# biointec/columba

Hardware: AMD Instinct MI355X
Metric: reads/sec (150bp, k=4 edit, human ref) (higher is better)
Workload: dtype u64

## Files before the change

### columba_amd/csrc/columba_amd.hip

```cpp
#include "../../include/columba_amd.h"
#include "host_sam.hpp"
#include "host_schemes.hpp"
#include "kernels.hpp"

#include <chrono>
#include <cstring>
#include <functional>
#include <memory>
#include <mutex>
#include <thread>
#include <string>
#include <vector>

using namespace cmb;

static thread_local std::string g_err;
static int fail(int code, const std::string& msg) {
    g_err = msg;
    return code;
}
namespace cmb {
int failWith(int code, const std::string& msg) { return fail(code, msg); }
}
#define HIPCHK(expr)                                                                                  \
    do {                                                                                              \
        hipError_t _e = (expr);                                                                       \
        if (_e != hipSuccess) throw std::runtime_error(std::string(#expr) + ": " + hipGetErrorString(_e)); \
    } while (0)

template <typename T> struct DevBuf {
    T* p = nullptr;
    size_t n = 0;
    DevBuf() {}
    DevBuf(const DevBuf&) = delete;
    DevBuf& operator=(const DevBuf&) = delete;
    ~DevBuf() { release(); }
    void release() {
        if (p) (void)hipFree(p);
        p = nullptr;
        n = 0;
    }
    void alloc(size_t count) {
        release();
        if (count == 0) count = 1;
        HIPCHK(hipMalloc((void**)&p, count * sizeof(T)));
        n = count;
    }
    void upload(const T* h, size_t count) {
        alloc(count);
        if (count) HIPCHK(hipMemcpy(p, h, count * sizeof(T), hipMemcpyHostToDevice));
    }
    void uploadPadded(const T* h, size_t count, size_t pad) {
        alloc(count + pad);
        if (count) HIPCHK(hipMemcpy(p, h, count * sizeof(T), hipMemcpyHostToDevice));
        HIPCHK(hipMemset(p + count, 0, pad * sizeof(T)));
    }
    size_t bytes() const { return n * sizeof(T); }
};

template <typename T> struct PinnedBuf {
    T* p = nullptr;
    size_t cap = 0, n = 0;
    PinnedBuf() {}
    PinnedBuf(const PinnedBuf&) = delete;
    PinnedBuf& operator=(const PinnedBuf&) = delete;
    ~PinnedBuf() {
        if (p) (void)hipHostFree(p);
    }
    void resize(size_t count) {
        if (count > cap) {
            if (p) (void)hipHostFree(p);
            p = nullptr;
            cap = 0;
            const size_t want = count + count / 4 + 64;
            HIPCHK(hipHostMalloc((void**)&p, want * sizeof(T), hipHostMallocDefault));
            cap = want;
        }
        n = count;
    }
    size_t size() const { return n; }
    bool empty() const { return n == 0; }
    T* data() { return p; }
    const T* data() const { return p; }
};

struct cmb_index {
    int device = 0;
    uint32_t saSparseness = 0;
    DevIndex d{};
    DevBuf<uint4> blkF, blkR;
    DevBuf<uint32_t> saSamples;
    DevBuf<uint8_t> text;
    DevBuf<uint32_t> text2;
    DevBuf<uint4> kmer;
    std::vector<uint32_t> seqStarts;
    DevBuf<uint32_t> seqStartsDev;
    uint32_t nSeqsDev = 0;
    uint64_t bytes = 0;
    bool textOnly = false;
    void uploadSeqStarts() {
        std::vector<uint32_t> v = seqStarts;
        if (v.size() < 2) v = {0u, d.n ? d.n - 1u : 0u};
        seqStartsDev.upload(v.data(), v.size());
        nSeqsDev = (uint32_t)v.size() - 1u;
    }
};

#ifdef CMB_BFS_STATS
extern "C" int cmb_debug_bfs_stats(unsigned long long* out, int reset) {
    if (out && hipMemcpyFromSymbol(out, HIP_SYMBOL(cmb::g_bfsStats), 16 * sizeof(unsigned long long)) != hipSuccess) return -1;
    if (reset) {
        unsigned long long z[16] = {};
        if (hipMemcpyToSymbol(HIP_SYMBOL(cmb::g_bfsStats), z, sizeof(z)) != hipSuccess) return -1;
    }
    return 0;
}
#endif
#ifdef CMB_BOUNDS
extern "C" int cmb_debug_oob(unsigned long long* out) {
    return hipMemcpyFromSymbol(out, HIP_SYMBOL(cmb::g_oob), 4 * sizeof(unsigned long long)) == hipSuccess ? 0 : -1;
}
#endif
#ifdef CMB_STAGE_STATS
extern "C" int cmb_debug_stage_stats(unsigned long long* out, int reset) {
    if (out && hipMemcpyFromSymbol(out, HIP_SYMBOL(cmb::g_stageStats), 24 * sizeof(unsigned long long)) != hipSuccess) return -1;
    if (reset) {
        unsigned long long z[24] = {};
        if (hipMemcpyToSymbol(HIP_SYMBOL(cmb::g_stageStats), z, sizeof(z)) != hipSuccess) return -1;
    }
    return 0;
}
#endif
extern "C" const char* cmb_last_error(void) { return g_err.c_str(); }
extern "C" const char* cmb_version(void) { return "columba_amd 0.1 (gfx950)"; }

static void useDevice(int device) { HIPCHK(hipSetDevice(device)); }

static int probeIndex(cmb_index* ix) {
    DevBuf<uint32_t> bad;
    bad.alloc(1);
    HIPCHK(hipMemset(bad.p, 0, sizeof(uint32_t)));
    const uint32_t nProbe = std::min<uint32_t>(ix->d.n, 1u << 20);
    if (!nProbe) return CMB_OK;
    hipLaunchKernelGGL(k_check_index, dim3((nProbe + 255) / 256), dim3(256), 0, 0, ix->d, ix->saSparseness, nProbe, (uint32_t)std::min<size_t>(ix->saSamples.n, 0xFFFFFFFFu), bad.p);
    HIPCHK(hipGetLastError());
    uint32_t hb = 0;
    HIPCHK(hipMemcpy(&hb, bad.p, sizeof(uint32_t), hipMemcpyDeviceToHost));
    if (hb)
        return fail(CMB_ERR_INVALID, "the index arrays do not belong together: " + std::to_string(hb) + " of " + std::to_string(nProbe) +
                                         " probed suffix-array rows do not reach a sampled row within " + std::to_string(ix->saSparseness) +
                                         " LF steps (wrong sparseness, or bit vectors / samples / BWT of different texts)");
    return CMB_OK;
}
extern "C" int cmb_index_validate(cmb_index* idx) {
    if (!idx) return fail(CMB_ERR_INVALID, "null argument");
    try {
        useDevice(idx->device);
        return probeIndex(idx);
    } catch (const std::exception& e) {
        return fail(CMB_ERR_DEVICE, e.what());
    }
}

extern "C" int cmb_index_create(const cmb_index_desc* desc, int device, cmb_index** out) {
    if (!desc || !out) return fail(CMB_ERR_INVALID, "null argument");
    if (desc->text_length == 0 || desc->text_length >= 0xFFFFFFFFull)
        return fail(CMB_ERR_UNSUPPORTED, "text length must fit a 32-bit length_t");
    if (desc->kmer_size > 15) return fail(CMB_ERR_INVALID, "k-mer size > 15 (the reference's -K option takes 0 ... 15, alignparameters.cpp:449)");
    if (desc->sa_sparseness == 0 || (desc->sa_sparseness & (desc->sa_sparseness - 1)))
        return fail(CMB_ERR_INVALID, "suffix array sparseness must be a power of two");
    try {
        int ndev = 0;
        if (hipGetDeviceCount(&ndev) != hipSuccess || ndev == 0)
            return fail(CMB_ERR_DEVICE, "no HIP device available (the product path has no CPU fallback)");
        useDevice(device);
        std::unique_ptr<cmb_index> ix(new cmb_index());
        ix->device = device;
        ix->saSparseness = desc->sa_sparseness;
        const uint64_t n = desc->text_length, N = n + 1;
        const uint64_t bvW = 4 * ((N + 63) / 64), cW = 8 * ((N + 511) / 512);
        const uint64_t nBlocks = N / RANK_BLOCK + 1;
        for (int dir = 0; dir < 2; dir++) {
            DevBuf<uint64_t> bv, cnt;
            bv.upload(dir ? desc->bv_rev : desc->bv_fwd, bvW);
            cnt.upload(dir ? desc->cnt_rev : desc->cnt_fwd, cW);
            DevBuf<uint4>& blk = dir ? ix->blkR : ix->blkF;
            blk.alloc(nBlocks * 2);
            hipLaunchKernelGGL(k_relayout, dim3((unsigned)((nBlocks + 255) / 256)), dim3(256), 0, 0, bv.p, cnt.p, N,
                               nBlocks, blk.p);
            HIPCHK(hipGetLastError());
            HIPCHK(hipDeviceSynchronize());
        }
        const uint64_t saW = (n + 63) / 64;
        {
            DevBuf<uint64_t> bv, cnt;
            bv.upload(desc->sa_bv, saW);
            cnt.upload(desc->sa_bv_counts, (saW + 7) / 4);
            hipLaunchKernelGGL(k_relayout_sa, dim3((unsigned)((nBlocks + 255) / 256)), dim3(256), 0, 0, bv.p, cnt.p, saW,
                               nBlocks, ix->blkF.p);
            HIPCHK(hipGetLastError());
            HIPCHK(hipDeviceSynchronize());
        }
        ix->saSamples.upload(desc->sa_samples, desc->n_samples);
        constexpr uint64_t TEXT_PAD = 640;
        static_assert(TEXT_PAD >= (uint64_t)VROWS + 64, "text padding must cover the longest verification window");
        ix->text.alloc(n + TEXT_PAD);
        HIPCHK(hipMemset(ix->text.p, 0, n + TEXT_PAD));
        HIPCHK(hipMemcpy(ix->text.p, desc->text, n, hipMemcpyHostToDevice));
        hipLaunchKernelGGL(k_encode_text, dim3(4096), dim3(256), 0, 0, ix->text.p, n, n + TEXT_PAD);
        HIPCHK(hipGetLastError());
        bool packedOk = false;
        {
            const uint64_t nWords = (n + TEXT_PAD) / 16;
            ix->text2.alloc(nWords + 16);
            HIPCHK(hipMemset(ix->text2.p, 0, (nWords + 16) * sizeof(uint32_t)));
            DevBuf<uint32_t> bad;
            bad.alloc(1);
            HIPCHK(hipMemset(bad.p, 0, sizeof(uint32_t)));
            hipLaunchKernelGGL(k_pack_text, dim3(4096), dim3(256), 0, 0, ix->text.p, n, nWords, ix->text2.p, bad.p);
            HIPCHK(hipGetLastError());
            uint32_t hb = 0;
            HIPCHK(hipMemcpy(&hb, bad.p, sizeof(uint32_t), hipMemcpyDeviceToHost));
            packedOk = hb == 0 && !getenv("CMB_TEXT_BYTES");
            if (!packedOk) ix->text2.release();
        }
        ix->kmer.alloc(1ull << (2 * desc->kmer_size));
        if (desc->seq_starts) ix->seqStarts.assign(desc->seq_starts, desc->seq_starts + desc->n_seqs);
        DevIndex& d = ix->d;
        d.n = (uint32_t)n;
        for (int i = 0; i < 5; i++) d.counts[i] = (uint32_t)desc->counts[i];
        d.fwd = DevBWT{ix->blkF.p, (uint32_t)desc->dollar_pos_fwd};
        d.rev = DevBWT{ix->blkR.p, (uint32_t)desc->dollar_pos_rev};
        d.saSamples = ix->saSamples.p;
        d.text = ix->text.p;
        d.text2 = packedOk ? ix->text2.p : nullptr;
        d.kmer = ix->kmer.p;
        d.kmerSize = desc->kmer_size;
        d.switchPoint = desc->in_text_switch;
        const uint32_t total = 1u << (2 * desc->kmer_size);
        hipLaunchKernelGGL(k_kmer_table, dim3((total + 255) / 256), dim3(256), 0, 0, d, ix->kmer.p);
        HIPCHK(hipGetLastError());
        HIPCHK(hipDeviceSynchronize());
        if (int rc = probeIndex(ix.get())) return rc;
        ix->bytes = ix->blkF.bytes() + ix->blkR.bytes() + ix->saSamples.bytes() + ix->text.bytes() + ix->text2.bytes() + ix->kmer.bytes();
        ix->uploadSeqStarts();
        *out = ix.release();
        return CMB_OK;
    } catch (const std::exception& e) {
        return fail(CMB_ERR_DEVICE, e.what());
    }
}
namespace {
struct ArrayRef {
    void** p;
    size_t* n;
    size_t elem;
};
inline void indexArrays(cmb_index* ix, ArrayRef out[CMB_DEV_ARRAYS]) {
    out[0] = {(void**)&ix->blkF.p, &ix->blkF.n, sizeof(uint4)};
    out[1] = {(void**)&ix->blkR.p, &ix->blkR.n, sizeof(uint4)};
    out[2] = {(void**)&ix->saSamples.p, &ix->saSamples.n, sizeof(uint32_t)};
    out[3] = {(void**)&ix->text.p, &ix->text.n, sizeof(uint8_t)};
    out[4] = {(void**)&ix->text2.p, &ix->text2.n, sizeof(uint32_t)};
    out[5] = {(void**)&ix->kmer.p, &ix->kmer.n, sizeof(uint4)};
}
inline void bindDevIndex(cmb_index* ix) {
    DevIndex& d = ix->d;
    d.fwd.blk = ix->blkF.p;
    d.rev.blk = ix->blkR.p;
    d.saSamples = ix->saSamples.p;
    d.text = ix->text.p;
    d.text2 = ix->text2.n ? ix->text2.p : nullptr;
    d.kmer = ix->kmer.p;
}
}

extern "C" int cmb_index_layout_of(const cmb_index* idx, cmb_index_layout* out) {
    if (!idx || !out) return fail(CMB_ERR_INVALID, "null argument");
    memset(out, 0, sizeof(*out));
    out->text_length = idx->d.n;
    for (int i = 0; i < 5; i++) out->counts[i] = idx->d.counts[i];
    out->dollar_pos_fwd = idx->d.fwd.dollarPos;
    out->dollar_pos_rev = idx->d.rev.dollarPos;
    out->n_samples = idx->saSamples.n;
    out->sa_sparseness = idx->saSparseness;
    out->kmer_size = idx->d.kmerSize;
    out->in_text_switch = idx->d.switchPoint;
    out->n_seqs = (uint32_t)idx->seqStarts.size();
    ArrayRef a[CMB_DEV_ARRAYS];
    indexArrays(const_cast<cmb_index*>(idx), a);
    for (int i = 0; i < CMB_DEV_ARRAYS; i++) out->bytes[i] = *a[i].p ? (uint64_t)(*a[i].n * a[i].elem) : 0;
    return CMB_OK;
}
extern "C" int cmb_index_seq_starts(const cmb_index* idx, uint32_t* out) {
    if (!idx || (!out && !idx->seqStarts.empty())) return fail(CMB_ERR_INVALID, "null argument");
    if (!idx->seqStarts.empty()) memcpy(out, idx->seqStarts.data(), idx->seqStarts.size() * sizeof(uint32_t));
    return CMB_OK;
}
extern "C" int cmb_index_create_text_only(const char* text, uint64_t n, const uint32_t* seq_starts, uint32_t n_seqs, int device,
                                          cmb_index** out) {
    if (!text || !out) return fail(CMB_ERR_INVALID, "null argument");
    if (n == 0 || n >= 0xFFFFFF00ull) return fail(CMB_ERR_UNSUPPORTED, "text length must fit a 32-bit length_t");
    try {
        useDevice(device);
        std::unique_ptr<cmb_index> ix(new cmb_index());
        ix->device = device;
        ix->textOnly = true;
        constexpr uint64_t TEXT_PAD = 640;
        ix->text.alloc(n + TEXT_PAD);
        HIPCHK(hipMemset(ix->text.p, 0, n + TEXT_PAD));
        HIPCHK(hipMemcpy(ix->text.p, text, n, hipMemcpyHostToDevice));
        hipLaunchKernelGGL(k_encode_text, dim3(4096), dim3(256), 0, 0, ix->text.p, n, n + TEXT_PAD);
        const uint64_t nWords = (n + TEXT_PAD) / 16;
        ix->text2.alloc(nWords + 16);
        HIPCHK(hipMemset(ix->text2.p, 0, (nWords + 16) * sizeof(uint32_t)));
        DevBuf<uint32_t> bad;
        bad.alloc(1);
        HIPCHK(hipMemset(bad.p, 0, sizeof(uint32_t)));
        hipLaunchKernelGGL(k_pack_text, dim3(4096), dim3(256), 0, 0, ix->text.p, n, nWords, ix->text2.p, bad.p);
        HIPCHK(hipGetLastError());
        uint32_t hb = 0;
        HIPCHK(hipMemcpy(&hb, bad.p, sizeof(uint32_t), hipMemcpyDeviceToHost));
        if (hb) ix->text2.release();
        if (seq_starts && n_seqs) ix->seqStarts.assign(seq_starts, seq_starts + n_seqs);
        ix->d.n = (uint32_t)n;
        ix->d.text = ix->text.p;
        ix->d.text2 = hb ? nullptr : ix->text2.p;
        ix->uploadSeqStarts();
        ix->bytes = ix->text.bytes() + ix->text2.bytes();
        *out = ix.release();
        return CMB_OK;
    } catch (const std::exception& e) {
        return fail(CMB_ERR_DEVICE, e.what());
    }
}

extern "C" int cmb_index_create_empty(const cmb_index_layout* L, const uint32_t* seq_starts, int device, cmb_index** out) {
    if (!L || !out) return fail(CMB_ERR_INVALID, "null argument");
    if (L->text_length == 0 || L->text_length >= 0xFFFFFFFFull || L->kmer_size > 15)
        return fail(CMB_ERR_INVALID, "index layout out of range");
    try {
        int ndev = 0;
        if (hipGetDeviceCount(&ndev) != hipSuccess || ndev == 0)
            return fail(CMB_ERR_DEVICE, "no HIP device available (the product path has no CPU fallback)");
        useDevice(device);
        std::unique_ptr<cmb_index> ix(new cmb_index());
        ix->device = device;
        ix->saSparseness = L->sa_sparseness;
        ArrayRef a[CMB_DEV_ARRAYS];
        indexArrays(ix.get(), a);
        {
            const uint64_t n = L->text_length, rankBytes = ((n + 1) / RANK_BLOCK + 1) * 2 * sizeof(uint4);
            if (L->sa_sparseness == 0 || (L->sa_sparseness & (L->sa_sparseness - 1)))
// ... 2433 lines not shown
```

### columba_amd/csrc/dev_index.hpp

```cpp
#pragma once
#include <hip/hip_runtime.h>
#include <stdint.h>

namespace cmb {

struct DevBWT {
    const uint4* blk;
    uint32_t dollarPos;
};

struct DevIndex {
    uint32_t n;
    uint32_t counts[5];
    DevBWT fwd, rev;
    const uint32_t* saSamples;
    const uint8_t* text;
    const uint32_t* text2;
    const uint4* kmer;
    uint32_t kmerSize;
    uint32_t switchPoint;
};

struct Range {
    uint32_t b, e;
    __host__ __device__ bool empty() const { return e <= b; }
    __host__ __device__ uint32_t width() const { return e <= b ? 0u : e - b; }
};
struct RangePair {
    Range sa, rev;
    __host__ __device__ bool empty() const { return sa.empty(); }
    __host__ __device__ uint32_t width() const { return sa.width(); }
};

constexpr uint32_t RANK_BLOCK = 32;

struct RankChunks {
    uint4 abs, bits;
    uint32_t bit;
};
__device__ __forceinline__ void loadRankChunks(const DevBWT& t, uint32_t p, RankChunks& k) {
    const uint4* B = t.blk + (size_t)(p >> 5) * 2;
    k.bit = p & 31u;
    k.abs = B[0];
    k.bits = B[1];
}
__device__ __forceinline__ void ranksFromChunks(const RankChunks& k, uint32_t p, uint32_t dollarPos, uint32_t R[4]) {
    const uint32_t lowmask = (1u << k.bit) - 1u;
    R[0] = k.abs.x + (uint32_t)__popc(k.bits.x & lowmask);
    R[1] = k.abs.y + (uint32_t)__popc(k.bits.y & lowmask);
    R[2] = k.abs.z + (uint32_t)__popc(k.bits.z & lowmask);
    R[3] = p - (p > dollarPos ? 1u : 0u);
}

__device__ __forceinline__ void loadRankChunksRaw(const DevBWT& t, uint32_t p, uint4 v[2]) {
    const uint4* B = t.blk + (size_t)(p >> 5) * 2;
    v[0] = B[0];
    v[1] = B[1];
}
__device__ __forceinline__ void loadRankPairRaw(const DevBWT& t, uint32_t pb, uint32_t pe, uint4 v[4]) {
    const uint32_t blkB = pb >> 5, blkE = pe >> 5;
    const uint4* B = t.blk + (size_t)blkB * 2;
    const uint4* E = t.blk + (size_t)blkE * 2;
    v[0] = B[0];
    v[1] = B[1];
    v[2] = v[3] = make_uint4(0u, 0u, 0u, 0u);
    if (blkE != blkB) {
        v[2] = E[0];
        v[3] = E[1];
    }
}
__device__ __forceinline__ void rankPairEnd(const uint4 v[4], uint32_t pb, uint32_t pe, uint4 w[2]) {
    const bool same = (pb >> 5) == (pe >> 5);
    w[0] = same ? v[0] : v[2];
    w[1] = same ? v[1] : v[3];
}
__device__ __forceinline__ void ranksFromRaw(const uint4 v[2], uint32_t p, uint32_t dollarPos, uint32_t R[4]) {
    const uint32_t lowmask = (1u << (p & 31u)) - 1u;
    R[0] = v[0].x + (uint32_t)__popc(v[1].x & lowmask);
    R[1] = v[0].y + (uint32_t)__popc(v[1].y & lowmask);
    R[2] = v[0].z + (uint32_t)__popc(v[1].z & lowmask);
    R[3] = p - (p > dollarPos ? 1u : 0u);
}

__device__ __forceinline__ void rank4(const DevBWT& t, uint32_t p, uint32_t R[4]) {
    RankChunks k;
    loadRankChunks(t, p, k);
    ranksFromChunks(k, p, t.dollarPos, R);
}

__device__ __forceinline__ uint64_t rank1(const DevBWT& t, uint32_t c, uint64_t p) {
    uint32_t R[4];
    rank4(t, (uint32_t)p, R);
    return R[c];
}

__device__ __forceinline__ uint32_t rankRefLayout(const uint64_t* bv, const uint64_t* cnt, uint32_t c, uint64_t p,
                                                  uint64_t N) {
    uint32_t extra = 0;
// ... 39 lines not shown
    r2.e = s + x + r1.width();
    if (mode == 1) {
        child.sa = r1;
        child.rev = r2;
    } else {
        child.sa = r2;
        child.rev = r1;
    }
    return !child.sa.empty();
}

__device__ __forceinline__ bool childFromRanksFlat(const DevIndex& ix, int mode, const RangePair& p, uint32_t c, const uint32_t Rb[4],
                                                   const uint32_t Re[4], uint32_t db, uint32_t de, RangePair& child) {
    const uint32_t start = ix.counts[c];
    const uint32_t b1 = occFromR(Rb, c) + start, e1 = occFromR(Re, c) + start;
    const uint32_t w1 = e1 > b1 ? e1 - b1 : 0u;
    const uint32_t x = cumFromR(Re, c, de) - cumFromR(Rb, c, db);
    const uint32_t b2 = (mode == 1 ? p.rev.b : p.sa.b) + x, e2 = b2 + w1;
    const bool fwd = mode == 0, uni = mode == 2;
    child.sa.b = fwd ? b2 : b1;
    child.sa.e = fwd ? e2 : e1;
    child.rev.b = uni ? 0u : fwd ? b1 : b2;
    child.rev.e = uni ? 0u : fwd ? e1 : e2;
    return e1 > b1;
}

__device__ __forceinline__ void loadExtendRanks(const DevIndex& ix, int mode, const RangePair& p,
                                                uint32_t Rb[4], uint32_t Re[4], uint32_t& db,
                                                uint32_t& de) {
    DevBWT t = ix.fwd;
    Range tr = p.sa;
    if (mode == 0) {
        t = ix.rev;
        tr = p.rev;
    }
    uint4 v[4], w[2];
    loadRankPairRaw(t, tr.b, tr.e, v);
    rankPairEnd(v, tr.b, tr.e, w);
    ranksFromRaw(v, tr.b, t.dollarPos, Rb);
    ranksFromRaw(w, tr.e, t.dollarPos, Re);
    db = tr.b > t.dollarPos ? 1u : 0u;
    de = tr.e > t.dollarPos ? 1u : 0u;
}

__device__ __forceinline__ bool extendOne(const DevIndex& ix, int mode, const RangePair& p, uint32_t c,
                                          RangePair& child) {
    uint32_t Rb[4], Re[4], db, de;
    loadExtendRanks(ix, mode, p, Rb, Re, db, de);
    return childFromRanks(ix, mode, p, c, Rb, Re, db, de, child);
}

__device__ __forceinline__ bool rowSampled(const RankChunks& k) { return (k.bits.w >> k.bit) & 1u; }
__device__ __forceinline__ uint32_t sampleIndex(const RankChunks& k) {
    return k.abs.w + (uint32_t)__popc(k.bits.w & ((1u << k.bit) - 1u));
}
__device__ __forceinline__ bool saMarked(const DevIndex& ix, uint32_t row) {
    RankChunks k;
    loadRankChunks(ix.fwd, row, k);
    return rowSampled(k);
}
__device__ __forceinline__ uint32_t saRank(const DevIndex& ix, uint32_t row) {
    RankChunks k;
    loadRankChunks(ix.fwd, row, k);
    return sampleIndex(k);
}

__device__ __forceinline__ uint32_t lfFromChunks(const DevIndex& ix, const RankChunks& ch, uint32_t k) {
    if (k == ix.fwd.dollarPos) {
        return ix.counts[0];
    }
    uint32_t R[4];
    ranksFromChunks(ch, k, ix.fwd.dollarPos, R);
    const uint32_t bit = ch.bit;
    const uint32_t c = ((ch.bits.x >> bit) & 1u) ? 1u : ((ch.bits.y >> bit) & 1u) ? 2u : ((ch.bits.z >> bit) & 1u) ? 3u : 4u;
    return ix.counts[c] + occFromR(R, c);
}
__device__ __forceinline__ uint32_t findLF(const DevIndex& ix, uint32_t k) {
    if (k == ix.fwd.dollarPos) return ix.counts[0];
    RankChunks ch;
    loadRankChunks(ix.fwd, k, ch);
    return lfFromChunks(ix, ch, k);
}

__device__ __forceinline__ uint32_t findSA(const DevIndex& ix, uint32_t row, uint32_t* lf) {
    uint32_t l = 0;
    RankChunks ch;
    loadRankChunks(ix.fwd, row, ch);
    while (!rowSampled(ch)) {
        row = lfFromChunks(ix, ch, row);
        loadRankChunks(ix.fwd, row, ch);
        l++;
    }
    if (lf) *lf += l;
    return ix.saSamples[sampleIndex(ch)] + l;
}

}
```

### columba_amd/csrc/kernels.hpp

```cpp
#pragma once
#include "dev_partition.hpp"
#include <cstring>
#include <rocprim/device/device_radix_sort.hpp>
#include <rocprim/device/device_scan.hpp>
#include <rocprim/device/device_run_length_encode.hpp>

namespace cmb {

__global__ void k_rank(DevIndex ix, int rev, const uint32_t* __restrict__ c, const uint64_t* __restrict__ p,
                       uint64_t n, uint64_t* __restrict__ out) {
    const uint64_t i = (uint64_t)blockIdx.x * blockDim.x + threadIdx.x;
    if (i >= n) return;
    out[i] = rank1(rev ? ix.rev : ix.fwd, c[i], p[i]);
}

__device__ __forceinline__ uint32_t rank9RefLayout(const uint64_t* bv, const uint64_t* cnt, uint64_t nWords, uint64_t p) {
    uint64_t w = p >> 6, b = p & 63;
    if (nWords == 0) return 0;
    if (w >= nWords) {
        w = nWords - 1;
        b = 64;
    }
    uint64_t rv = cnt[(w >> 3) * 2];
    const uint32_t sub = (uint32_t)(w & 7u);
    if (sub) rv += (cnt[(w >> 3) * 2 + 1] >> ((sub - 1u) * 9u)) & 0x1FFull;
    const uint64_t lowmask = b >= 64 ? ~0ull : b ? (~0ull >> (64 - b)) : 0ull;
    return (uint32_t)rv + (uint32_t)__popcll((unsigned long long)(bv[w] & lowmask));
}

__global__ void k_relayout(const uint64_t* __restrict__ bv, const uint64_t* __restrict__ cnt, uint64_t N,
                           uint64_t nBlocks, uint4* __restrict__ out) {
    const uint64_t blk = (uint64_t)blockIdx.x * blockDim.x + threadIdx.x;
    if (blk >= nBlocks) return;
    const uint64_t nWords = (N + 63) / 64;
    const uint64_t w = blk >> 1;
    const uint32_t sh = (uint32_t)(blk & 1u) * 32u;
    uint32_t bits[3];
    for (uint32_t c = 0; c < 3; c++) bits[c] = w < nWords ? (uint32_t)(bv[w * 4 + c] >> sh) : 0u;
    uint4 abs;
    abs.x = rankRefLayout(bv, cnt, 0, blk * RANK_BLOCK, N);
    abs.y = rankRefLayout(bv, cnt, 1, blk * RANK_BLOCK, N);
    abs.z = rankRefLayout(bv, cnt, 2, blk * RANK_BLOCK, N);
    abs.w = 0;
    out[blk * 2] = abs;
    out[blk * 2 + 1] = make_uint4(bits[0], bits[1], bits[2], 0u);
}

__global__ void k_relayout_sa(const uint64_t* __restrict__ saBv, const uint64_t* __restrict__ saCnt, uint64_t saWords, uint64_t nBlocks,
                              uint4* __restrict__ out) {
    const uint64_t blk = (uint64_t)blockIdx.x * blockDim.x + threadIdx.x;
    if (blk >= nBlocks) return;
    const uint64_t w = blk >> 1;
    const uint32_t sh = (uint32_t)(blk & 1u) * 32u;
    reinterpret_cast<uint32_t*>(out + blk * 2)[3] = rank9RefLayout(saBv, saCnt, saWords, blk * RANK_BLOCK);
    reinterpret_cast<uint32_t*>(out + blk * 2 + 1)[3] = w < saWords ? (uint32_t)(saBv[w] >> sh) : 0u;
}

__global__ void __launch_bounds__(256)
k_extend(DevIndex ix, int mode, const uint4* __restrict__ in, uint64_t n, uint4* __restrict__ out,
         uint8_t* __restrict__ ok) {
    for (uint64_t i = (uint64_t)blockIdx.x * blockDim.x + threadIdx.x; i < n;
         i += (uint64_t)gridDim.x * blockDim.x) {
        const uint4 v = in[i];
        RangePair p{{v.x, v.y}, {v.z, v.w}};
        uint32_t Rb[4], Re[4], db, de;
        loadExtendRanks(ix, mode, p, Rb, Re, db, de);
        uint32_t okbits = 0;
#pragma unroll
        for (uint32_t ch = 1; ch <= 4; ch++) {
            RangePair child;
            const bool o = childFromRanks(ix, mode, p, ch, Rb, Re, db, de, child);
            out[i * 4 + (ch - 1)] = make_uint4(child.sa.b, child.sa.e, child.rev.b, child.rev.e);
            okbits |= (o ? 1u : 0u) << (8 * (ch - 1));
        }
        reinterpret_cast<uint32_t*>(ok)[i] = okbits;
    }
}

__global__ void k_locate(DevIndex ix, const uint32_t* __restrict__ rows, uint64_t n, uint32_t* __restrict__ out,
                         unsigned long long* lfTotal) {
    const uint64_t i = (uint64_t)blockIdx.x * blockDim.x + threadIdx.x;
    if (i >= n) return;
    uint32_t lf = 0;
    out[i] = findSA(ix, rows[i], &lf);
    if (lf) atomicAdd(lfTotal, (unsigned long long)lf);
}

__global__ void k_check_index(DevIndex ix, uint32_t maxSteps, uint32_t nProbe, uint32_t nSamples, uint32_t* __restrict__ bad) {
    const uint32_t i = blockIdx.x * blockDim.x + threadIdx.x;
    if (i >= nProbe) return;
    uint32_t row = (uint32_t)(((uint64_t)i * ix.n) / nProbe);
    for (uint32_t l = 0;; l++) {
        if (row >= ix.n) break;
        RankChunks ch;
        loadRankChunks(ix.fwd, row, ch);
        if (rowSampled(ch)) {
            const uint32_t si = sampleIndex(ch);
            if (si < nSamples && (uint64_t)ix.saSamples[si] + l < ix.n) return;
            break;
        }
        if (l == maxSteps) break;
        row = lfFromChunks(ix, ch, row);
    }
    atomicAdd(bad, 1u);
}

__global__ void k_kmer_table(DevIndex ix, uint4* __restrict__ table) {
    const uint32_t key = blockIdx.x * blockDim.x + threadIdx.x;
    const uint32_t total = 1u << (2 * ix.kmerSize);
    if (key >= total) return;
    RangePair r{{0, ix.n}, {0, ix.n}};
    bool ok = true;
    for (int i = (int)ix.kmerSize - 1; i >= 0 && ok; i--) {
        const uint32_t code = ((key >> (2 * i)) & 3u) + 1u;
        RangePair child;
        ok = extendOne(ix, 0, r, code, child);
        r = child;
    }
    table[key] = ok ? make_uint4(r.sa.b, r.sa.e, r.rev.b, r.rev.e) : make_uint4(0, 0, 0, 0);
}

struct __attribute__((packed, aligned(1))) Unaligned16 {
    uint32_t x, y, z, w;
};
struct __attribute__((packed, aligned(1))) Unaligned8 {
    uint32_t x, y;
};
__device__ __forceinline__ uint4 loadText16(const uint8_t* p) {
    const Unaligned16 v = *reinterpret_cast<const Unaligned16*>(p);
    return make_uint4(v.x, v.y, v.z, v.w);
}
__global__ void __launch_bounds__(256)
k_prep(const uint8_t* __restrict__ reads, const uint64_t* __restrict__ offs, uint32_t nReads, uint32_t maxLen,
       uint32_t gw, uint32_t chunks, uint8_t* __restrict__ seq, uint32_t* __restrict__ G, uint32_t* __restrict__ rec,
       uint32_t recW) {
    const uint32_t gid = blockIdx.x * blockDim.x + threadIdx.x;
    const uint32_t r = gid / chunks, w = gid % chunks;
    if (r >= nReads) return;
    const uint8_t* rd = reads + offs[r];
    const uint32_t len = (uint32_t)(offs[r + 1] - offs[r]);
    if (len > maxLen) return;
    if (32 * w >= len) {
        if (w == 0 && rec) {
            rec[(size_t)(2 * r) * recW] = 0;
            rec[(size_t)(2 * r + 1) * recW] = 0;
        }
        return;
    }
    uint32_t fA[4] = {0, 0, 0, 0}, fB[4] = {0, 0, 0, 0};
    uint8_t* sF = seq + (size_t)(2 * r) * maxLen;
    uint8_t* sR = seq + (size_t)(2 * r + 1) * maxLen;
    const uint32_t nT = min(32u, len - 32 * w);
    uint32_t cF[8] = {0, 0, 0, 0, 0, 0, 0, 0}, cR[8] = {0, 0, 0, 0, 0, 0, 0, 0};
    uint32_t wa[8], wb[8];
    {
        const uint4 x = loadText16(rd + 32 * w), y = loadText16(rd + 32 * w + 16);
        wa[0] = x.x, wa[1] = x.y, wa[2] = x.z, wa[3] = x.w, wa[4] = y.x, wa[5] = y.y, wa[6] = y.z, wa[7] = y.w;
    }
    if (offs[r] + len >= 32ull * w + 32ull) {
        const uint8_t* pb = rd + len - 32 * w - 32;
        const uint4 x = loadText16(pb), y = loadText16(pb + 16);
        wb[0] = x.x, wb[1] = x.y, wb[2] = x.z, wb[3] = x.w, wb[4] = y.x, wb[5] = y.y, wb[6] = y.z, wb[7] = y.w;
    } else {
#pragma unroll
        for (uint32_t j = 0; j < 8; j++) wb[j] = 0;
#pragma unroll
        for (uint32_t t = 0; t < 32; t++)
            if (t < nT) wb[(31u - t) >> 2] |= (uint32_t)rd[len - 1 - 32 * w - t] << (8u * ((31u - t) & 3u));
// ... 544 lines not shown
            nxt = loadText16(tp + 16 * (c + 2));
        }
    }
    if (!STORE && i > firstRow) {
        const uint32_t e1 = edPrev;
        if (e1 <= maxED && e1 >= minED && e1 <= edPrev2) centreMask |= 1u << (i - 1 - firstRow);
    }
    return i;
}

constexpr uint32_t VK_LOW = 10;
__host__ __device__ __forceinline__ uint32_t windowEnd(uint32_t maxEnd, uint32_t start, uint32_t m) {
    const unsigned long long e = (unsigned long long)start + m - 1ull;
    return e < maxEnd ? (uint32_t)e : maxEnd;
}
__host__ __device__ __forceinline__ unsigned long long packVerifyKey(uint32_t rs, uint32_t start, uint32_t maxED,
                                                                     uint32_t minED, uint32_t fixed) {
    return ((unsigned long long)rs << 39) | ((unsigned long long)(maxED & 7u) << 36) | ((unsigned long long)(minED & 7u) << 33) |
           ((unsigned long long)(fixed & 1u) << 32) | (unsigned long long)((start >> VK_LOW) | (start << (32u - VK_LOW)));
}
__host__ __device__ __forceinline__ uint32_t verifyKeyStart(unsigned long long key) {
    const uint32_t v = (uint32_t)key;
    return (v << VK_LOW) | (v >> (32u - VK_LOW));
}
constexpr uint32_t VKW_RS = 41;
__host__ __device__ __forceinline__ unsigned long long packVerifyKeyW(uint32_t rs, uint32_t start, uint32_t maxED, uint32_t minED,
                                                                      uint32_t fixed) {
    return ((unsigned long long)rs << VKW_RS) | ((unsigned long long)(maxED & 15u) << 37) | ((unsigned long long)(minED & 15u) << 33) |
           ((unsigned long long)(fixed & 1u) << 32) | (unsigned long long)((start >> VK_LOW) | (start << (32u - VK_LOW)));
}

__device__ __forceinline__ bool verifyEdit(const DevIndex& ix, const uint64_t* offs, const MFull& mf,
                                           uint32_t rs, uint32_t start, uint32_t maxED, uint32_t minED, uint32_t fixed,
                                           uint32_t mult, uint32_t& cStarted, uint32_t& cRows, uint32_t& cText,
                                           uint32_t& cAbort, uint32_t& cCig, uint4& tbRec, uint64_t* Ml,
                                           uint32_t limitEnd = 0 ) {
    cStarted += mult;
    const uint32_t len = (uint32_t)(offs[(rs >> 1) + 1] - offs[rs >> 1]);
    const uint32_t nZeros = fixed ? 1u : 2u * maxED + 1u;
    MatGeom g;
    g.n = len + 1;
    g.maxED = maxED;
    g.Wv = nZeros - 1 + maxED;
    g.Wh = maxED;
    g.m = max(g.Wv + g.n, g.Wv + g.Wh + 1u);
    const uint32_t maxEnd = ix.n - 1;
    const uint32_t hEnd = limitEnd ? min(maxEnd, limitEnd) : windowEnd(maxEnd, start, g.m);
    const uint32_t size = hEnd > start ? hEnd - start : 0;
    if (!g.inFinalColumn(size)) return false;
    uint32_t mask = 0, rows = 0;
    uint64_t edPack, edPackHi;
    const VPlanes noPlanes{nullptr, 0, 0};
    const uint32_t i = forwardPass<false>(ix, mf, rs, g, nZeros, start, size, maxED, minED,
                                          mask, edPack, edPackHi, noPlanes, 0, rows, Ml);
    cRows += rows * mult;
    cText += rows * mult;
    if (i <= size - g.sfc() || mask == 0) {
        cAbort += mult;
        return false;
    }
    cCig += (uint32_t)__popc(mask) * mult;
    tbRec = make_uint4(rs, start, mask, maxED | (fixed << 4));
    return true;
}

__device__ __forceinline__ uint32_t mismatch4(uint32_t tw, uint32_t sw) {
    const uint32_t x = (tw + 0x01010101u) ^ sw;
    return ((x | (x >> 1) | (x >> 2)) | (tw >> 2)) & 0x01010101u;
}
__device__ __forceinline__ uint32_t mismatch16(const uint4& t, const uint4& r, uint32_t nC, uint32_t m[4]) {
    const uint32_t tw[4] = {t.x, t.y, t.z, t.w}, sw[4] = {r.x, r.y, r.z, r.w};
    uint32_t cnt = 0;
#pragma unroll
    for (uint32_t w = 0; w < 4; w++) {
        const uint32_t nb = nC > 4 * w ? min(4u, nC - 4 * w) : 0u;
        const uint32_t valid = nb >= 4u ? 0x01010101u : (0x01010101u & ((1u << (8u * nb)) - 1u));
        m[w] = mismatch4(tw[w], sw[w]) & valid;
        cnt += (uint32_t)__popc(m[w]);
    }
    return cnt;
}

template <bool KEYS>
__global__ void __launch_bounds__(256)
k_verify(DevIndex ix, const uint64_t* __restrict__ offs, uint32_t maxLen, uint32_t gw,
         const uint8_t* __restrict__ seq, MFull mf, const uint4* __restrict__ items,
         uint32_t nItems, uint4* __restrict__ tbq, uint32_t tbCap, unsigned long long* __restrict__ vkeys, Queues q,
         uint32_t wideKeys = 0 ) {
    __shared__ uint64_t Ml[ML_WORDS];
    const uint32_t slot = blockIdx.x * blockDim.x + threadIdx.x;
    uint32_t cLF = 0, cLoc = 0, cText = 0, cRows = 0, cAbort = 0, cCig = 0, cStarted = 0, cRep = 0, flags = 0;
    WaveChunk chT, chB;
    bool ovT = false, ovB = false;
    auto holeT = [&](uint32_t i) { q.text[i].rsId = 0xFFFFFFFFu; };
    auto holeB = [&](uint32_t i) { tbq[i] = make_uint4(0, 0, 0, 0); };
    const uint32_t stride = gridDim.x * blockDim.x;
    const uint32_t waveBase = slot & ~63u;
    const VPlanes noPlanes{nullptr, 0, 0};
    for (uint32_t base = waveBase; base < nItems; base += stride) {
        const uint32_t it = base + (threadIdx.x & 63u);
        uint32_t nOut = 0, nTb = 0;
        uint4 outRec = make_uint4(0, 0, 0, 0), tbRec = make_uint4(0, 0, 0, 0);
        uint32_t rs = 0;
        unsigned long long vkey = ~0ull;
        uint4 item = make_uint4(0xFFFFFFFFu, 0, 0, 0);
        if (it < nItems) item = items[it];
        if (item.x != 0xFFFFFFFFu) {
            rs = item.x;
            const uint32_t row = item.y, a = item.z, meta = item.w;
            const uint32_t kind = (meta >> 21) & 3u;
            const uint32_t maxED = (meta >> 12) & 15u, minED = (meta >> 16) & 15u;
            const uint32_t fixed = (meta >> 20) & 1u;
            const uint32_t shift = meta & 0xFFFu;
            const uint32_t len = (uint32_t)(offs[(rs >> 1) + 1] - offs[rs >> 1]);
            const uint8_t* s = seq + (size_t)rs * maxLen;
            uint32_t pos;
            if ((meta >> 23) & 1u) {
                pos = row;
            } else {
                cLoc++;
                pos = findSA(ix, row, &cLF);
            }
            if (kind == ITEM_EXACT) {
                if (fixed) {
                    outRec = make_uint4(pos, pos + len, 0, 0);
                    nOut = 1;
                } else {
                    cStarted++;
                    const uint32_t remaining = a;
                    bool ok = pos >= remaining;
                    const uint32_t p0 = pos - remaining;
                    for (uint32_t j = 0; ok && j < remaining; j += 16) {
                        const uint32_t nC = min(16u, remaining - j);
                        uint32_t m[4];
                        const uint32_t cnt = mismatch16(loadText16(ix.text + p0 + j), *reinterpret_cast<const uint4*>(s + j), nC, m);
                        if (cnt == 0) {
                            cText += nC;
                        } else {
                            const uint32_t w = m[0] ? 0u : m[1] ? 1u : m[2] ? 2u : 3u;
                            const uint32_t mw = w == 0 ? m[0] : w == 1 ? m[1] : w == 2 ? m[2] : m[3];
                            cText += 4 * w + (((uint32_t)__ffs(mw) - 1u) >> 3) + 1u;
                            ok = false;
                        }
                    }
                    if (ok) {
                        outRec = make_uint4(p0, p0 + len, 0, 0);
                        nOut = 1;
                    } else {
                        cAbort++;
                    }
                }
            } else if (kind == ITEM_HAMMING) {
                cStarted++;
                const uint32_t lengthBefore = a;
                const uint32_t Tb = pos > lengthBefore ? pos - lengthBefore : 0;
                const uint32_t Te = Tb + len;
                if ((unsigned long long)Tb + len <= ix.n) {
                    uint32_t score = 0;
                    for (uint32_t j = 0; j < len; j += 16) {
                        const uint32_t nC = min(16u, len - j);
                        uint32_t m[4];
                        const uint32_t cnt = mismatch16(loadText16(ix.text + Tb + j), *reinterpret_cast<const uint4*>(s + j), nC, m);
                        if (score + cnt <= maxED) {
                            score += cnt;
                            cText += nC;
                            continue;
                        }
                        for (uint32_t t = 0; t < nC; t++) {
                            const uint32_t mw = (t >> 2) == 0 ? m[0] : (t >> 2) == 1 ? m[1] : (t >> 2) == 2 ? m[2] : m[3];
                            cText++;
                            score += (mw >> (8u * (t & 3u))) & 1u;
                            if (score > maxED) break;
                        }
                        break;
                    }
                    if (score <= maxED && score >= minED) {
                        outRec = make_uint4(Tb, Te, score, 0);
                        nOut = 1;
                    }
                }
            } else {
                const bool direct = (meta >> 23) & 1u;
                const uint32_t startDiff = direct ? 0u : a;
                const uint32_t sum = pos + shift;
                const uint32_t start = sum >= startDiff ? sum - startDiff : 0;
                if (KEYS) {
                    vkey = wideKeys ? packVerifyKeyW(rs, start, maxED, minED, fixed) : packVerifyKey(rs, start, maxED, minED, fixed);
                } else if (verifyEdit(ix, offs, mf, rs, start, maxED, minED, fixed, 1u, cStarted, cRows, cText, cAbort,
                                      cCig, tbRec, Ml, direct ? a : 0u)) {
                    nTb = 1;
                }
            }
        }
        if (KEYS && it < nItems) vkeys[it] = vkey;
        cRep += nOut;
        const uint32_t o1 = chT.alloc(&q.cnt[2], q.textCap, nOut, 256u, ovT, holeT);
        if (nOut && o1 != 0xFFFFFFFFu) q.text[o1] = TextOccRec{rs, outRec.x, outRec.y, outRec.z};
        const uint32_t o2 = chB.alloc(&q.cnt[7], tbCap, nTb, 256u, ovB, holeB);
        if (nTb && o2 != 0xFFFFFFFFu) tbq[o2] = tbRec;
    }
    chT.fill(holeT);
    chB.fill(holeB);
    if (ovT) flags |= FLAG_TEXT_OVERFLOW;
    if (ovB) flags |= FLAG_CAPACITY;
// ... 122 lines not shown
            if (!__any(have)) {
                if (__all(done)) break;
                turn = 0xFFFFFFFFu;
                continue;
            }
            if (have) mx.loadBlock(ix, G, gw, rs, len, start, r >> 4);
            skip = fresh;
            if (fresh) r = 1u;
        }
        bool survives = false;
        if (have && !skip) {
            uint64_t M, D0;
            const bool valid = mx.step(g, r, M, D0);
            rows++;
            if (!valid || r == size) {
                const uint32_t i = valid ? r : r - 1u;
                if (i <= size - g.sfc()) {
                    cStarted += mult;
                    cRows += rows * mult;
                    cAbort += mult;
                } else {
                    survives = true;
                }
                have = false;
            } else {
                r++;
            }
        }
        if (__any(survives)) {
            const uint32_t o = chS.alloc(&work[1], listCap, survives ? 1u : 0u, 256u, ovS, holeS);
            if (survives && o != 0xFFFFFFFFu) list[o] = u;
        }
    }
    chS.fill(holeS);
    if (ovS) flags |= FLAG_CAPACITY;
    const uint32_t local[8] = {0u, 0u, cRows, cRows, cAbort, 0u, cStarted, 0u};
    const int which[8] = {8, 9, 10, 11, 3, 4, 2, 1};
    flushCounters(q, local, which, 8);
    if (flags) atomicOr(&q.cnt[3], flags);
}

template <bool KEYED, class WX>
__global__ void __launch_bounds__(256)
k_verify_wide(DevIndex ix, const uint64_t* __restrict__ offs, uint32_t maxLen, const uint8_t* __restrict__ seq, const uint32_t* __restrict__ G,
              uint32_t gw, const uint4* __restrict__ items, uint32_t nItems, const unsigned long long* __restrict__ ukeys,
              const uint32_t* __restrict__ counts, const uint32_t* __restrict__ list, const uint32_t* __restrict__ nList,
              uint8_t* __restrict__ slab, uint32_t slotBytes, Queues q) {
    const uint32_t slot = blockIdx.x * blockDim.x + threadIdx.x, nSlots = gridDim.x * blockDim.x, lane = threadIdx.x & 63u;
    uint4* const rowBits = reinterpret_cast<uint4*>(slab + (size_t)(slot - lane) * slotBytes) + lane;
    auto putRow = [&](uint32_t r, uint64_t a, uint64_t b) {
        rowBits[(size_t)r * 64u] = make_uint4((uint32_t)a, (uint32_t)(a >> 32), (uint32_t)b, (uint32_t)(b >> 32));
    };
    uint32_t cLF = 0, cLoc = 0, cRows = 0, cAbort = 0, cCig = 0, cStarted = 0, flags = 0;
    const uint32_t nIn = KEYED ? min(*nList, nItems) : nItems;
    WaveChunk chT;
    bool ovT = false;
    auto holeT = [&](uint32_t o) { q.text[o].rsId = 0xFFFFFFFFu; };
    for (uint32_t base = slot - lane; base < nIn; base += nSlots) {
        const uint32_t it = base + lane;
        bool active = it < nIn;
        uint32_t rs = 0, maxED = 0, minED = 0, fixed = 0, start = 0, limitEnd = 0u, mult = 1u;
        if (active && KEYED) {
            const uint32_t u = list[it];
            if (u == 0xFFFFFFFFu) {
                active = false;
            } else {
                const unsigned long long key = ukeys[u];
                mult = counts[u];
                rs = (uint32_t)(key >> VKW_RS), maxED = (uint32_t)(key >> 37) & 15u, minED = (uint32_t)(key >> 33) & 15u, fixed = (uint32_t)(key >> 32) & 1u;
                start = verifyKeyStart(key);
            }
        } else if (active) {
            const uint4 item = items[it];
            const uint32_t meta = item.w;
            if (item.x == 0xFFFFFFFFu || ((meta >> 21) & 3u) != ITEM_EDIT) {
                active = false;
            } else {
                rs = item.x, maxED = (meta >> 12) & 15u, minED = (meta >> 16) & 15u, fixed = (meta >> 20) & 1u;
                const uint32_t shift = meta & 0xFFFu;
                const bool direct = (meta >> 23) & 1u;
                uint32_t pos = item.y;
                if (!direct) {
                    cLoc++;
                    pos = findSA(ix, item.y, &cLF);
                }
                const uint32_t startDiff = direct ? 0u : item.z;
                limitEnd = direct ? item.z : 0u;
                const uint32_t sum = pos + shift;
                start = sum >= startDiff ? sum - startDiff : 0;
            }
        }
        const uint32_t len = active ? (uint32_t)(offs[(rs >> 1) + 1] - offs[rs >> 1]) : 0u;
        const uint8_t* rd = seq + (size_t)rs * maxLen;
        const uint32_t nZeros = fixed ? 1u : 2u * maxED + 1u;
        const MatGeom g = wideGeom(len, maxED, nZeros);
        const uint32_t sfc = g.sfc(), col = g.n - 1u, firstRow = (g.m - 1u) - sfc;
        unsigned long long lcw0 = 0ull, lcw1 = 0ull, lcw2 = 0ull, lcw3 = 0ull;
        auto lcPut = [&](uint32_t qi, uint32_t v) {
            const unsigned long long x = (unsigned long long)min(v, 15u) << (4u * (qi & 15u));
            lcw0 |= (qi >> 4) == 0u ? x : 0ull, lcw1 |= (qi >> 4) == 1u ? x : 0ull, lcw2 |= (qi >> 4) == 2u ? x : 0ull, lcw3 |= (qi >> 4) == 3u ? x : 0ull;
        };
        auto lcGet = [&](uint32_t qi) -> uint32_t {
            const unsigned long long w = (qi >> 4) == 0u ? lcw0 : (qi >> 4) == 1u ? lcw1 : (qi >> 4) == 2u ? lcw2 : lcw3;
            return (uint32_t)(w >> (4u * (qi & 15u))) & 15u;
        };
        uint32_t i = 0;
        if (active) {
            cStarted += mult;
            const uint32_t maxEnd = ix.n - 1;
            const uint32_t hEnd = limitEnd ? min(maxEnd, limitEnd) : windowEnd(maxEnd, start, g.m);
            const uint32_t size = hEnd > start ? hEnd - start : 0;
            if (!g.inFinalColumn(size)) {
                active = false;
            } else if (g.Wv >= WX::LEFT || (size + 1u) * VW_ROW_BYTES > slotBytes) {
                flags |= FLAG_CAPACITY;
                active = false;
            } else {
                WideRow<WX> mx;
                mx.init(g, nZeros);
                putRow(0u, mx.HP, ~0ull);
                if (firstRow == 0u) lcPut(0u, cellAt<WX::BLOCK, WX::DIAG>(0u, col, mx.HP, mx.HN, mx.score));
                for (uint32_t r = 1; r <= size; r++) {
                    if (r == 1u || (r & 15u) == 0u) mx.loadBlock(ix, G, gw, rs, len, start, r >> 4);
                    uint64_t M, D0;
                    const bool valid = mx.step(g, r, M, D0);
                    cRows += mult;
                    putRow(r, mx.HP, M | ~D0);
                    if (!valid) break;
                    if (r >= firstRow) lcPut(r - firstRow, cellAt<WX::BLOCK, WX::DIAG>(r, col, mx.HP, mx.HN, mx.score));
                    i = r;
                }
                if (i <= size - sfc) {
                    cAbort += mult;
                    active = false;
                }
            }
        }
        const uint32_t nCand = active && i > firstRow ? i - firstRow : 0u;
        uint32_t nCentres = 0;
        for (uint32_t t = 0; __any(t < nCand); t++) {
            bool emit = false;
            TextOccRec rec{0xFFFFFFFFu, 0u, 0u, 0u};
            if (t < nCand) {
                const uint32_t r = i - t;
                const uint32_t ED = lcGet(r - firstRow);
                if (ED <= maxED && ED >= minED) {
                    const bool betterThanAbove = r == firstRow || ED <= lcGet(r - 1u - firstRow);
                    const bool betterThanBelow = r == i || ED <= lcGet(r + 1u - firstRow);
                    if (betterThanAbove && betterThanBelow) {
                        nCentres++;
                        uint32_t ti = r, tj = col;
                        while (tj > 0) {
                            const uint32_t bitIdx = (tj - (ti / WX::BLOCK) * WX::BLOCK) + WX::DIAG;
                            if (bitIdx >= 64u) {
                                flags |= FLAG_CAPACITY;
                                break;
                            }
                            const uint4 rb = rowBits[(size_t)ti * 64u];
                            const uint64_t hp = rb.x | ((uint64_t)rb.y << 32), md = rb.z | ((uint64_t)rb.w << 32);
                            if ((hp >> bitIdx) & 1ull) {
                                --tj;
                            } else if (ti > 0 && ((md >> bitIdx) & 1ull)) {
                                --ti;
                                --tj;
                            } else if (ti > 0) {
                                --ti;
                            } else {
// ... 381 lines not shown
                        flags |= FLAG_CAPACITY;
                        break;
                    }
                    const bool hpBit = ((uint32_t)ww >> rel) & 1u;
                    const bool dgBit = ((uint32_t)(ww >> 32) >> rel) & 1u;
                    if (rel < relLeft || rel > relRight || (rel == relLeft && hpBit) ||
                        (rel == relRight && ti > 0 && !hpBit && !dgBit))
                        flags |= FLAG_TRACE_RULE;
                    if (hpBit) {
                        --tj;
                    } else {
                        if (ti > 0 && dgBit) --tj;
                        --ti;
                    }
                }
            }
            if (have) {
                const uint32_t ed = bitIdx < 21u ? (uint32_t)((edPack >> (3u * bitIdx)) & 7ull)
                                                 : (uint32_t)((edPackHi >> (3u * (bitIdx - 21u))) & 7ull);
                rec = TextOccRec{rs, start + ti, start + ri, ed};
            }
            const uint32_t o = chT.alloc(&q.cnt[2], q.textCap, have ? 1u : 0u, 256u, ovT, holeT);
            if (have && o != 0xFFFFFFFFu) q.text[o] = rec;
        }
    }
    chT.fill(holeT);
    if (ovT) flags |= FLAG_TEXT_OVERFLOW;
    if (flags) atomicOr(&q.cnt[3], flags);
}

__global__ void k_fm_keys(const FMOccRec* __restrict__ fm, uint32_t n, unsigned long long* __restrict__ keys,
                          uint32_t* __restrict__ idx) {
    const uint32_t i = blockIdx.x * blockDim.x + threadIdx.x;
    if (i >= n) return;
    const FMOccRec f = fm[i];
    keys[i] = f.rsId == 0xFFFFFFFFu ? ~0ull : (((unsigned long long)(f.rsId >> 1) << 32) | f.b);
    idx[i] = i;
}
__global__ void __launch_bounds__(256)
k_fm_unique(const FMOccRec* __restrict__ fm, const unsigned long long* __restrict__ keys, const uint32_t* __restrict__ idx,
            uint32_t n, FMOccRec* __restrict__ out, uint32_t* __restrict__ nOut, Queues q) {
    const uint32_t j = blockIdx.x * blockDim.x + threadIdx.x;
    bool keep = false;
    FMOccRec f{};
    if (j < n && keys[j] != ~0ull) {
        f = fm[idx[j]];
        keep = true;
        for (uint32_t t = j; t-- > 0 && keys[t] == keys[j];) {
            const FMOccRec g = fm[idx[t]];
            if (g.rsId == f.rsId && g.e == f.e && g.dist == f.dist && g.depth == f.depth && g.shift == f.shift) {
                keep = false;
                break;
            }
        }
    }
    uint32_t total;
    const uint32_t o = waveAppend(nOut, keep ? 1u : 0u, total);
    if (keep) out[o] = f;
    unsigned long long rows = keep ? (unsigned long long)(f.e - f.b) : 0ull;
#pragma unroll
    for (int d = 32; d >= 1; d >>= 1) rows += __shfl_xor(rows, d);
    if ((threadIdx.x & 63u) == 0 && rows) atomicAdd(&q.counters[1], rows);
}

__global__ void __launch_bounds__(256)
k_fmocc(DevIndex ix, const FMOccRec* __restrict__ recs, uint32_t n, Queues q) {
    uint32_t cLF = 0, cLoc = 0, flags = 0;
    const uint32_t stride = gridDim.x * blockDim.x;
    const uint32_t first = blockIdx.x * blockDim.x + threadIdx.x;
    for (uint32_t base = first & ~63u; base < n; base += stride) {
        const uint32_t i = base + (threadIdx.x & 63u);
        FMOccRec f{};
        uint32_t w = 0;
        if (i < n) {
            f = recs[i];
            w = f.e - f.b;
        }
        uint32_t total;
        const uint32_t o = waveAppend(&q.cnt[2], w, total);
        if (o + w > q.textCap) {
            if (w) flags |= FLAG_TEXT_OVERFLOW;
            continue;
        }
        for (uint32_t t = 0; t < w; t++) {
            cLoc++;
            const uint32_t p = findSA(ix, f.b + t, &cLF) + f.shift;
            q.text[o + t] = TextOccRec{f.rsId, p, p + f.depth, f.dist};
        }
    }
    const uint32_t local[2] = {cLF, cLoc};
    const int which[2] = {8, 9};
    flushCounters(q, local, which, 2);
    if (flags) atomicOr(&q.cnt[3], flags);
}

__global__ void __launch_bounds__(256)
k_pack_keys(const TextOccRec* __restrict__ text, uint32_t n, const uint64_t* __restrict__ offs, uint32_t k,
            unsigned long long* __restrict__ keys, uint32_t* __restrict__ cnt,
            uint32_t perStrand ,
            const uint8_t* __restrict__ only = nullptr ,
            uint32_t layout = 0 ) {
    const uint32_t i = blockIdx.x * blockDim.x + threadIdx.x;
    if (i >= n) return;
    const TextOccRec t = text[i];
    if (t.rsId == 0xFFFFFFFFu || (only && !(only[t.rsId] & 0x80u))) {
        keys[i] = ~0ull;
        return;
    }
    const uint32_t r = t.rsId >> 1;
    const uint32_t len = (uint32_t)(offs[r + 1] - offs[r]);
    const uint32_t width = t.end - t.begin;
    const uint32_t wrel = width - (len - k);
    const uint32_t grp = perStrand ? t.rsId : r;
    const KeyBits kb = keyBits(layout);
    uint32_t low;
    if (layout == 1u) {
        if (width != len || t.dist > kb.distMask) atomicOr(&cnt[3], (uint32_t)FLAG_CAPACITY);
        low = (t.dist & kb.distMask) << kb.dist;
    } else {
        if (wrel > kb.wMask || t.dist > kb.distMask) atomicOr(&cnt[3], (uint32_t)FLAG_CAPACITY);
        low = ((t.dist & kb.distMask) << kb.dist) | ((wrel & kb.wMask) << 1);
    }
    if ((unsigned long long)grp >> (64u - kb.group)) atomicOr(&cnt[3], (uint32_t)FLAG_CAPACITY);
    keys[i] = ((unsigned long long)grp << kb.group) | ((unsigned long long)t.begin << kb.begin) | (unsigned long long)low |
              (unsigned long long)(perStrand ? 0u : (t.rsId & 1u));
}

__global__ void k_filter_segments(const unsigned long long* __restrict__ keys, uint32_t n, uint32_t* __restrict__ segBeg,
                                  uint32_t* __restrict__ segEnd, uint32_t groupShift = 40u) {
    const uint32_t i = blockIdx.x * blockDim.x + threadIdx.x;
    if (i >= n) return;
    const unsigned long long key = keys[i];
    if (key == ~0ull) return;
    const uint32_t r = (uint32_t)(key >> groupShift);
    if (i == 0 || (uint32_t)(keys[i - 1] >> groupShift) != r) segBeg[r] = i;
    if (i + 1 == n || keys[i + 1] == ~0ull || (uint32_t)(keys[i + 1] >> groupShift) != r) segEnd[r] = i + 1;
}

constexpr uint32_t FILTER_NONE = 0xFFFFFFFFu;
constexpr uint32_t FILTER_SHORT = 24;
__global__ void __launch_bounds__(256)
k_filter_mark(const unsigned long long* __restrict__ keys, uint32_t nReads, uint32_t k, int mode,
              uint32_t* __restrict__ counts, uint32_t* __restrict__ rank, const uint32_t* __restrict__ segBeg,
              const uint32_t* __restrict__ segEnd, uint32_t layout = 0u) {
    const KeyBits kb = keyBits(layout);
    const uint32_t r = blockIdx.x * blockDim.x + threadIdx.x;
    const uint32_t lane = threadIdx.x & 63u;
    uint32_t segLo = 0xFFFFFFFFu;
    if (r < nReads) segLo = segBeg[r];
    const bool has = segLo != 0xFFFFFFFFu;
    const uint32_t nSeg = has ? segEnd[r] - segLo : 0u;
    const uint32_t maxDiff = 2 * k;
    struct State {
        uint32_t nOut = 0, lastKept = 0, prevBegin = 0xFFFFFFFFu, prevDepth = 0xFFFFFFFFu, prevED;
        unsigned long long prevKey = ~0ull;
    };
    auto stepCore = [&](State& st, uint32_t i, unsigned long long key, uint32_t& replaced) -> uint32_t {
        const uint32_t begin = (uint32_t)(key >> kb.begin), dist = (uint32_t)(key >> kb.dist) & kb.distMask;
        const uint32_t width = (uint32_t)(key >> 1) & kb.wMask;
        replaced = FILTER_NONE;
        bool keep = true;
        if (mode != 0) {
            if ((key >> 1) == (st.prevKey >> 1)) keep = false;
            else st.prevKey = key;
        }
        if (keep && mode == 2) {
// ... 365 lines not shown
```

Baseline: 54.42 million.

## Materialize dense suffix array on device to replace LF-walk locates

At index build or validate time, when enough device memory is free, a new kernel expands the sampled suffix array into a full dense SA by running a checked findSA for every row. All locate sites (k_verify, k_fmocc, the locate kernel) then read saDense[row] directly instead of walking LF steps. The LF counters are kept consistent by deriving the step count from the position's low bits. In exchange this uses about 4n bytes of extra device memory (around 12 GB for a human reference) and adds build time. The diff also sets a min-waves occupancy hint on the KEYS variant of k_verify.

```diff
diff --git a/columba_amd/csrc/columba_amd.hip b/columba_amd/csrc/columba_amd.hip
--- a/columba_amd/csrc/columba_amd.hip
+++ b/columba_amd/csrc/columba_amd.hip
@@ -90,6 +90,7 @@
     DevIndex d{};
     DevBuf<uint4> blkF, blkR;
     DevBuf<uint32_t> saSamples;
+    DevBuf<uint32_t> saDense;
     DevBuf<uint8_t> text;
     DevBuf<uint32_t> text2;
     DevBuf<uint4> kmer;
@@ -152,11 +153,41 @@
                                          " LF steps (wrong sparseness, or bit vectors / samples / BWT of different texts)");
     return CMB_OK;
 }
+static void buildDenseSA(cmb_index* ix) {
+    ix->bytes -= ix->saDense.bytes();
+    ix->saDense.release();
+    ix->d.saDense = nullptr;
+    const uint64_t n = ix->d.n;
+    if (getenv("CMB_SA_SPARSE") || n == 0 || ix->saSparseness == 0 || !ix->saSamples.p || !ix->d.fwd.blk) return;
+    size_t freeB = 0, totalB = 0;
+    HIPCHK(hipMemGetInfo(&freeB, &totalB));
+    uint64_t minFree = std::min<uint64_t>(128ull << 30, totalB / 2);
+    if (const char* e = getenv("CMB_TEST_SA_MIN_FREE_GB")) minFree = (uint64_t)(atof(e) * (double)(1ull << 30));
+    if (freeB < n * sizeof(uint32_t) || freeB - n * sizeof(uint32_t) < minFree) return;
+    ix->saDense.alloc(n);
+    DevBuf<uint32_t> bad;
+    bad.alloc(1);
+    HIPCHK(hipMemset(bad.p, 0, sizeof(uint32_t)));
+    const uint32_t nSamples = (uint32_t)std::min<size_t>(ix->saSamples.n, 0xFFFFFFFFu);
+    hipLaunchKernelGGL(k_dense_sa, dim3((unsigned)std::min<uint64_t>((n + 255) / 256, 1u << 16)), dim3(256), 0, 0, ix->d, nSamples,
+                       ix->saDense.p, bad.p);
+    HIPCHK(hipGetLastError());
+    uint32_t hb = 0;
+    HIPCHK(hipMemcpy(&hb, bad.p, sizeof(uint32_t), hipMemcpyDeviceToHost));
+    if (hb) {
+        ix->saDense.release();
+        return;
+    }
+    ix->d.saDense = ix->saDense.p;
+    ix->bytes += ix->saDense.bytes();
+}
 extern "C" int cmb_index_validate(cmb_index* idx) {
     if (!idx) return fail(CMB_ERR_INVALID, "null argument");
     try {
         useDevice(idx->device);
-        return probeIndex(idx);
+        if (int rc = probeIndex(idx)) return rc;
+        buildDenseSA(idx);
+        return CMB_OK;
     } catch (const std::exception& e) {
         return fail(CMB_ERR_DEVICE, e.what());
     }
@@ -232,6 +263,7 @@
         d.fwd = DevBWT{ix->blkF.p, (uint32_t)desc->dollar_pos_fwd};
         d.rev = DevBWT{ix->blkR.p, (uint32_t)desc->dollar_pos_rev};
         d.saSamples = ix->saSamples.p;
+        d.saSparseness = ix->saSparseness;
         d.text = ix->text.p;
         d.text2 = packedOk ? ix->text2.p : nullptr;
         d.kmer = ix->kmer.p;
@@ -243,6 +275,7 @@
         HIPCHK(hipDeviceSynchronize());
         if (int rc = probeIndex(ix.get())) return rc;
         ix->bytes = ix->blkF.bytes() + ix->blkR.bytes() + ix->saSamples.bytes() + ix->text.bytes() + ix->text2.bytes() + ix->kmer.bytes();
+        buildDenseSA(ix.get());
         ix->uploadSeqStarts();
         *out = ix.release();
         return CMB_OK;
@@ -269,6 +302,8 @@
     d.fwd.blk = ix->blkF.p;
     d.rev.blk = ix->blkR.p;
     d.saSamples = ix->saSamples.p;
+    d.saDense = ix->saDense.n ? ix->saDense.p : nullptr;
+    d.saSparseness = ix->saSparseness;
     d.text = ix->text.p;
     d.text2 = ix->text2.n ? ix->text2.p : nullptr;
     d.kmer = ix->kmer.p;
diff --git a/columba_amd/csrc/dev_index.hpp b/columba_amd/csrc/dev_index.hpp
--- a/columba_amd/csrc/dev_index.hpp
+++ b/columba_amd/csrc/dev_index.hpp
@@ -14,6 +14,8 @@
     uint32_t counts[5];
     DevBWT fwd, rev;
     const uint32_t* saSamples;
+    const uint32_t* saDense;
+    uint32_t saSparseness;
     const uint8_t* text;
     const uint32_t* text2;
     const uint4* kmer;
@@ -219,17 +221,30 @@
     return lfFromChunks(ix, ch, k);
 }
 
-__device__ __forceinline__ uint32_t findSA(const DevIndex& ix, uint32_t row, uint32_t* lf) {
+template <bool CHECKED = false>
+__device__ __forceinline__ uint32_t findSA(const DevIndex& ix, uint32_t row, uint32_t* lf, uint32_t nSamples = 0) {
     uint32_t l = 0;
     RankChunks ch;
     loadRankChunks(ix.fwd, row, ch);
     while (!rowSampled(ch)) {
+        if (CHECKED && l == ix.saSparseness) return 0xFFFFFFFFu;
         row = lfFromChunks(ix, ch, row);
+        if (CHECKED && row >= ix.n) return 0xFFFFFFFFu;
         loadRankChunks(ix.fwd, row, ch);
         l++;
     }
+    if (CHECKED && sampleIndex(ch) >= nSamples) return 0xFFFFFFFFu;
     if (lf) *lf += l;
     return ix.saSamples[sampleIndex(ch)] + l;
 }
 
-}
+__device__ __forceinline__ uint32_t locateRow(const DevIndex& ix, uint32_t row, uint32_t* lf) {
+    if (ix.saDense) {
+        const uint32_t p = ix.saDense[row];
+        if (lf) *lf += p & (ix.saSparseness - 1u);
+        return p;
+    }
+    return findSA(ix, row, lf);
+}
+
+}
diff --git a/columba_amd/csrc/kernels.hpp b/columba_amd/csrc/kernels.hpp
--- a/columba_amd/csrc/kernels.hpp
+++ b/columba_amd/csrc/kernels.hpp
@@ -82,8 +82,20 @@
     const uint64_t i = (uint64_t)blockIdx.x * blockDim.x + threadIdx.x;
     if (i >= n) return;
     uint32_t lf = 0;
-    out[i] = findSA(ix, rows[i], &lf);
+    out[i] = locateRow(ix, rows[i], &lf);
     if (lf) atomicAdd(lfTotal, (unsigned long long)lf);
+}
+
+__global__ void __launch_bounds__(256) k_dense_sa(DevIndex ix, uint32_t nSamples, uint32_t* __restrict__ sa, uint32_t* __restrict__ bad) {
+    uint32_t nBad = 0;
+    const uint64_t stride = (uint64_t)gridDim.x * blockDim.x;
+    for (uint64_t row = (uint64_t)blockIdx.x * blockDim.x + threadIdx.x; row < ix.n; row += stride) {
+        uint32_t l = 0;
+        const uint32_t p = findSA<true>(ix, (uint32_t)row, &l, nSamples);
+        sa[row] = p;
+        nBad += (p >= ix.n || l != (p & (ix.saSparseness - 1u))) ? 1u : 0u;
+    }
+    if (nBad) atomicAdd(bad, nBad);
 }
 
 __global__ void k_check_index(DevIndex ix, uint32_t maxSteps, uint32_t nProbe, uint32_t nSamples, uint32_t* __restrict__ bad) {
@@ -794,7 +806,7 @@
 }
 
 template <bool KEYS>
-__global__ void __launch_bounds__(256)
+__global__ void __launch_bounds__(256, KEYS ? 8 : 1)
 k_verify(DevIndex ix, const uint64_t* __restrict__ offs, uint32_t maxLen, uint32_t gw,
          const uint8_t* __restrict__ seq, MFull mf, const uint4* __restrict__ items,
          uint32_t nItems, uint4* __restrict__ tbq, uint32_t tbCap, unsigned long long* __restrict__ vkeys, Queues q,
@@ -831,7 +843,7 @@
                 pos = row;
             } else {
                 cLoc++;
-                pos = findSA(ix, row, &cLF);
+                pos = locateRow(ix, row, &cLF);
             }
             if (kind == ITEM_EXACT) {
                 if (fixed) {
@@ -1120,7 +1132,7 @@
                 uint32_t pos = item.y;
                 if (!direct) {
                     cLoc++;
-                    pos = findSA(ix, item.y, &cLF);
+                    pos = locateRow(ix, item.y, &cLF);
                 }
                 const uint32_t startDiff = direct ? 0u : item.z;
                 limitEnd = direct ? item.z : 0u;
@@ -1668,6 +1680,22 @@
             if (w) flags |= FLAG_TEXT_OVERFLOW;
             continue;
         }
+        if (ix.saDense) {
+            for (uint32_t t = 0; t < w; t += 4) {
+                uint32_t sa[4];
+#pragma unroll
+                for (uint32_t j = 0; j < 4; j++) sa[j] = t + j < w ? ix.saDense[f.b + t + j] : 0u;
+#pragma unroll
+                for (uint32_t j = 0; j < 4; j++) {
+                    if (t + j >= w) break;
+                    cLF += sa[j] & (ix.saSparseness - 1u);
+                    const uint32_t p = sa[j] + f.shift;
+                    q.text[o + t + j] = TextOccRec{f.rsId, p, p + f.depth, f.dist};
+                }
+            }
+            cLoc += w;
+            continue;
+        }
         for (uint32_t t = 0; t < w; t++) {
             cLoc++;
             const uint32_t p = findSA(ix, f.b + t, &cLF) + f.shift;
```

New measurement: 58.65 million (median of 6 runs). 7.8% higher.
